# santurini/vsrlab

Hardware: AMD Instinct MI355X
Metric: LR frames/sec fwd+bwd, BasicVSR 4x 540p 7-frame clip, 1->8 MI355X (higher is better)
Workload: dtype bf16; 1 GPU; BasicVSR(mid=64,res_blocks=30,x4) fwd+Charbonnier+bwd+clip+Adam, 540x960->2160x3840, 7-frame clip, 2 clips per GPU (BASELINE configs[1]); clips_per_gpu=2, frames=7, res_blocks=30, parallelism=single GPU, arena=full, train_flow=False, trunk_chains=True

## Files before the change

vsrlab_amd/_lib.py:

```python
import ctypes
import os
from ctypes import c_char_p, c_float, c_int, c_longlong, c_size_t, c_void_p

_HERE = os.path.dirname(os.path.abspath(__file__))
LIB_PATH = os.environ.get("VSRLAB_AMD_LIB") or os.path.join(_HERE, "lib", "libvsrlab_hip.so")

DT_F32 = 0
DT_BF16 = 1


class BasicVSRDesc(ctypes.Structure):
    _fields_ = [("n", c_int), ("t", c_int), ("h", c_int), ("w", c_int), ("mid_channels", c_int),
                ("res_blocks", c_int), ("upscale", c_int), ("dtype", c_int), ("arena_mode", c_int)]


class DiscDesc(ctypes.Structure):
    _fields_ = [("n", c_int), ("h", c_int), ("w", c_int), ("mid_ch", c_int), ("dtype", c_int)]


class PerceptualDesc(ctypes.Structure):
    _fields_ = [("n", c_int), ("h", c_int), ("w", c_int), ("dtype", c_int), ("need_grad", c_int)]


class AttnDesc(ctypes.Structure):
# ... 101 lines not shown
    "vsr_raft_corr_lookup_fwd": (c_int, [ctypes.POINTER(RaftCorrDesc), _P, c_size_t, _P, _P, _P]),
    "vsr_raft_corr_lookup_bwd": (c_int, [ctypes.POINTER(RaftCorrDesc), _P, c_size_t, _P, _P, _P, c_size_t, _P]),
}
EXPORTS = tuple(_SIGNATURES)

OTHER_DEBUG_EXPORTS = ("vsr_debug_chain_inject_error", "vsr_debug_chain_item", "vsr_debug_chain_timeouts", "vsr_debug_chain_timing_begin",
                       "vsr_debug_chain_timing_read", "vsr_debug_warp_bwd_gather", "vsr_debug_warp_bwd_gather_c")
_LL = c_longlong
DEBUG_SIGNATURES = {
    "vsr_debug_tail_last2_fwd": (c_int, [c_int, _P, _P, _P, _P, _P, _P, _LL, _P, _P, _LL, c_int, c_int, c_int, c_int, c_int, c_int, c_int, _P]),
    "vsr_debug_tail_last2_dgrad": (c_int, [_P, _LL, _P, _P, c_int, _P, c_int, c_float, _P, c_int, c_int, c_int, _P]),
    "vsr_debug_tail_planar_c64": (c_int, [c_int, _P, _LL, c_int, _P, _P, _P, _P, c_int, c_float, _P, c_int, c_int, c_int, c_int, _P]),
    "vsr_debug_tail_last2_wgrad": (c_int, [c_int, _P, _P, _LL, c_int, _P, _P, _P, c_int, c_int, c_int, _P]),
    "vsr_debug_tail_conv_unshuffle": (c_int, [c_int, _P, _P, _P, c_int, _P, _P, c_int, c_int, c_int, _P]),
    "vsr_debug_tail_ps_dgrad": (c_int, [c_int, _P, _P, _P, _P, _P, c_int, c_int, _P, c_int, c_int, c_int, c_int, c_int, _P]),
    "vsr_debug_tail_ps_wgrads": (c_int, [c_int, _P, _P, c_int, _P, _P, _P, c_int, c_int, c_int, _P]),
    "vsr_debug_trunk_conv": (c_int, [c_int, c_int, c_int, c_int, _P, _P, _P, _P, _P, c_int, c_float, _P, _P, c_int, _P, _P, c_int, c_int,
                                     c_int, c_int, c_int, _P]),
    "vsr_debug_trunk_stem": (c_int, [c_int, c_int, c_int, _P, _P, _LL, _P, _P, _P, _P, c_int, c_float, c_int, c_int, c_int, _P]),
    "vsr_debug_trunk_stem_dgrad": (c_int, [c_int, c_int, c_int, _P, _P, _P, _P, _P, _LL, c_int, c_int, c_int, c_int, _P]),
    "vsr_debug_trunk_point": (c_int, [c_int, c_int, c_int, _P, _P, _P, _P, _P, _P, _P, c_int, c_int, c_int, _P]),
    "vsr_debug_trunk_wgrad_cc": (c_int, [c_int, c_int, c_int, _P, _P, c_int, _P, c_int, c_int, _P, c_int, _P, c_int, c_int, c_int, _P]),
    "vsr_debug_trunk_stem_wgrads": (c_int, [c_int, c_int, c_int, _P, _LL, _P, c_int, _P, _P, c_int, _P, _P, c_int, _P, c_int, c_int, c_int, _P]),
    "vsr_debug_trunk_chain": (c_int, [c_int, c_int, _P, _P, _P, c_int, _P, c_int, c_int, c_int, c_int, _P]),
    "vsr_debug_spy_conv": (c_int, [c_int, c_int, _P, _P, _P, _P, _P, c_int, _P, c_int, c_int, c_int, _P]),
    "vsr_debug_spy_dgrad": (c_int, [c_int, c_int, _P, _P, _P, _P, _P, c_int, c_int, c_int, _P]),
    "vsr_debug_spy_wgrad": (c_int, [c_int, c_int, _P, _P, _P, _P, c_int, _P, c_int, c_int, c_int, _P]),
    "vsr_debug_spy_prepare": (c_int, [c_int, _P, _P, _P, _P, c_int, c_int, c_int, c_int, c_int, c_int, c_int, _P]),
    "vsr_debug_spy_prepare_bwd": (c_int, [c_int, _P, _P, _P, _P, _P, _P, c_int, c_int, c_int, c_int, c_int, c_int, _P]),
    "vsr_debug_spy_dres": (c_int, [c_int, _P, _P, _P, c_int, c_int, c_int, _P]),
    "vsr_debug_spy_planar": (c_int, [c_int, _P, _P, _P, _P, _P, _LL, c_int, c_int, c_int, c_int, _P]),
}

SPATIAL_CORR_LIB_PATH = os.path.join(_HERE, "lib", "libvsrlab_spatial_corr.so")
SPATIAL_CORR_SIGNATURES = {
    "vsr_spatial_corr_workspace_bytes": (c_size_t, [ctypes.POINTER(SpatialCorrDesc)]),
    "vsr_spatial_corr_fwd": (c_int, [ctypes.POINTER(SpatialCorrDesc), _P, _P, _P, _P, c_size_t, _P]),
    "vsr_spatial_corr_bwd": (c_int, [ctypes.POINTER(SpatialCorrDesc), _P, _P, _P, _P, _P, _P, c_size_t, _P]),
}
SPATIAL_CORR_EXPORTS = tuple(SPATIAL_CORR_SIGNATURES)

JPEG_LIB_PATH = os.path.join(_HERE, "lib", "libvsrlab_jpeg.so")
JPEG_SIGNATURES = {
    "vsr_jpeg_workspace_bytes": (c_size_t, [ctypes.POINTER(JpegDesc)]),
    "vsr_jpeg_fwd": (c_int, [ctypes.POINTER(JpegDesc), _P, _P, _P, c_size_t, _P]),
}
JPEG_EXPORTS = tuple(JPEG_SIGNATURES)

WARP_TAPS_LIB_PATH = os.path.join(_HERE, "lib", "libvsrlab_warp_taps.so")
WARP_TAPS_SIGNATURES = {
    "vsr_warp_taps_fwd": (c_int, [ctypes.POINTER(WarpTapsDesc), _P, _P, _P, _P]),
    "vsr_warp_taps_bwd": (c_int, [ctypes.POINTER(WarpTapsDesc), _P, _P, _P, _P, _P]),
    "vsr_warp_taps_clip_fwd": (c_int, [ctypes.POINTER(WarpTapsDesc), _P, _P, _P, _P, _P]),
    "vsr_warp_taps_clip_bwd": (c_int, [ctypes.POINTER(WarpTapsDesc), _P, _P, _P, _P, _P, _P]),
}
WARP_TAPS_EXPORTS = tuple(WARP_TAPS_SIGNATURES)

_lib = None
_spatial_corr_lib = None
_jpeg_lib = None
_warp_taps_lib = None


def load_warp_taps():
    global _warp_taps_lib
    if _warp_taps_lib is None:
        if not os.path.exists(WARP_TAPS_LIB_PATH):
            raise RuntimeError(
                f"vsrlab_amd: HIP library not built ({WARP_TAPS_LIB_PATH} missing). Run "
                "`python -c 'import __graft_entry__ as g; g.build()'` or `make -C vsrlab_amd/csrc`.")
        lib = ctypes.CDLL(WARP_TAPS_LIB_PATH)
        for name, (res, args) in WARP_TAPS_SIGNATURES.items():
            fn = getattr(lib, name)
            fn.restype = res
            fn.argtypes = args
        _warp_taps_lib = lib
    return _warp_taps_lib


def load_jpeg():
    global _jpeg_lib
    if _jpeg_lib is None:
        if not os.path.exists(JPEG_LIB_PATH):
            raise RuntimeError(
                f"vsrlab_amd: HIP library not built ({JPEG_LIB_PATH} missing). Run "
                "`python -c 'import __graft_entry__ as g; g.build()'` or `make -C vsrlab_amd/csrc`.")
        lib = ctypes.CDLL(JPEG_LIB_PATH)
        for name, (res, args) in JPEG_SIGNATURES.items():
            fn = getattr(lib, name)
            fn.restype = res
            fn.argtypes = args
        _jpeg_lib = lib
    return _jpeg_lib

# ... 43 lines not shown
```

vsrlab_amd/csrc/conv3x3_persist.hip:

```cpp
#include "conv3x3_c64_tile.h"
#include <type_traits>

namespace {

constexpr int P_LDS = BIAS_OFF + 256;

__device__ uint4 g_conv_zero_chunk[2];

template <int ACT> __device__ __forceinline__ float p_act(float v, float slope) {
    if (ACT == ACT_RELU) return v > 0.f ? v : 0.f;
    if (ACT == ACT_LEAKY) return v > 0.f ? v : slope * v;
    return v;
}

#ifdef VSR_CLOCK
__device__ unsigned long long g_clk[256 * 4];
#endif

__device__ __forceinline__ void tile_coords(int tile, int ntx, int nty, int& n, int& ty0, int& tx0) {
    const int per = ntx * nty;
    n = tile / per;
    const int r = tile - n * per;
    const int ty = r / ntx;
    ty0 = ty * PTH;
    tx0 = (r - ty * ntx) * PTW;
}

struct TileIter {
    int tile, n, ty, tx;
    int sn, sty, stx;
    __device__ __forceinline__ void init(int first, int stride, int ntx, int nty) {
        const int per = ntx * nty;
        tile = first; n = first / per; int r = first - n * per; ty = r / ntx; tx = r - ty * ntx;
        sn = stride / per; r = stride - sn * per; sty = r / ntx; stx = r - sty * ntx;
    }
    __device__ __forceinline__ void advance(int stride, int ntx, int nty) {
        tile += stride;
        tx += stx; if (tx >= ntx) { tx -= ntx; ++ty; }
        ty += sty; if (ty >= nty) { ty -= nty; ++n; }
        n += sn;
    }
};

__device__ __forceinline__ float bf_lo(unsigned w) { return __uint_as_float(w << 16); }
__device__ __forceinline__ float bf_hi(unsigned w) { return __uint_as_float(w & 0xffff0000u); }

constexpr int DMA_PLAIN = 0;

template <int ACT, bool HAS_RES, int MASK>
__global__ __launch_bounds__(PNT, 1) void conv3x3_c64_persist_kernel(const ConvArgs ka) {
    extern __shared__ __attribute__((aligned(16))) char smem[];

    const int z = blockIdx.y;
    struct {
        int N, H, W, Ws, Wd, in_step, out_step, src_ox0, src_oy0, out_oxz, out_oyz, bias_zstride, unshuffle;
        long long src_nstride0, dst_nstride, w_zstride, plane;
        unsigned long long src0, wpack, resz, auxz, sign_bitsz, dstz, sign_outz, bias; float leaky_slope;
    } a = {ka.N, ka.H, ka.W, ka.Ws, ka.Wd, ka.in_step, ka.out_step, ka.src_ox[0], ka.src_oy[0], ka.out_ox[z], ka.out_oy[z], ka.bias_zstride, ka.unshuffle,
           ka.src_nstride[0], ka.dst_nstride, ka.w_zstride, ka.unshuffle_plane,
           (unsigned long long)ka.src[0], (unsigned long long)ka.wpack, (unsigned long long)ka.res[z], (unsigned long long)ka.aux[z],
           (unsigned long long)ka.sign_bits[z], (unsigned long long)ka.dst[z], (unsigned long long)ka.sign_out[z], (unsigned long long)ka.bias, ka.leaky_slope};
    asm volatile("" : "+s"(a.N), "+s"(a.H), "+s"(a.W), "+s"(a.Ws), "+s"(a.Wd), "+s"(a.in_step), "+s"(a.out_step), "+s"(a.src_ox0), "+s"(a.src_oy0),
                 "+s"(a.out_oxz), "+s"(a.out_oyz), "+s"(a.bias_zstride), "+s"(a.unshuffle), "+s"(a.src_nstride0), "+s"(a.dst_nstride), "+s"(a.w_zstride), "+s"(a.plane));
    asm volatile("" : "+s"(a.src0), "+s"(a.wpack), "+s"(a.resz), "+s"(a.auxz), "+s"(a.sign_bitsz), "+s"(a.dstz), "+s"(a.sign_outz), "+s"(a.bias), "+s"(a.leaky_slope));
    const int tid = threadIdx.x, lane = tid & 63, wave = tid >> 6;
    const int role = __builtin_amdgcn_readfirstlane(wave >> 2);
    const int w4 = wave & 3;
    const int l15 = lane & 15, q = lane >> 4;
    const int pxl = PM_LANE_PIXEL(l15);
    char* lds_w = smem;
    char* lds_t = smem + W_BYTES;
#ifdef VSR_CLOCK
    unsigned long long clk_t0 = 0, clk_r0 = 0;
    if (tid == 0) { clk_t0 = __builtin_amdgcn_s_memtime(); clk_r0 = __builtin_amdgcn_s_memrealtime(); }
#endif

    const int ntx = cdiv(a.W, PTW), nty = cdiv(a.H, PTH);
    const int total = a.N * ntx * nty;
    const int WSs = pm_ws(a.Ws), WSd = pm_ws(a.Wd);
    const TileWalk walk = xcd_tile_walk(total, blockIdx.x, gridDim.x);

    if (tid < 64) reinterpret_cast<float*>(smem + BIAS_OFF)[tid] = a.bias ? GP(const float, a.bias)[(long long)z * a.bias_zstride + pm_acc_chan(tid >> 4, tid & 15)] : 0.f;

    const auto* wg = GP(const u32x4_t, a.wpack + (unsigned long long)((long long)z * a.w_zstride) * 2);

    if (role == 1) {
        const auto* src = GP(const char, a.src0);
        const auto* zsrc = GP(const char, g_conv_zero_chunk);
        int rel[NPIECE_W];
        C64_DMA_REL(rel, w4, lane, a.in_step, a.src_oy0, a.src_ox0, WSs)
        auto issue = [&](const TileIter& it, int buf) {
            const int n = it.n, ty0 = it.ty * PTH, tx0 = it.tx * PTW;
            const auto* org = src + ((long long)n * a.src_nstride0 + pm_off(ty0 * a.in_step, tx0 * a.in_step, 0, a.Ws, 64)) * 2;
            char* dstb = lds_t + buf * IN_BYTES;
            C64_DMA_TILE(DMA_PLAIN, rel, org, zsrc, dstb, w4, lane, ty0, tx0, a.H, a.W)
        };
        int cur = 0;
        TileIter it;
        it.init(walk.first, walk.stride, ntx, nty);
        if (it.tile < walk.end) issue(it, 0);
        asm volatile("s_waitcnt vmcnt(0)" ::: "memory");
        __syncthreads();
        while (it.tile < walk.end) {
            it.advance(walk.stride, ntx, nty);
            if (it.tile < walk.end) issue(it, cur ^ 1);
            asm volatile("s_waitcnt vmcnt(0)" ::: "memory");
            __syncthreads();
            cur ^= 1;
        }
    } else {
        u32x4_t wv[WCH];
        C64_W_LOAD(wv, wg, tid)
        C64_MFMA_LANE(w4, l15, q, pxl)
        int loff[4];
#pragma unroll
        for (int nb = 0; nb < 4; ++nb) {
            const int dx = ((nb & 1) * 16 + pxl) * a.out_step + a.out_oxz;
            loff[nb] = ((((w4 * 2 + (nb >> 1)) * a.out_step) * WSd + (dx >> 5)) * 8 + q) * 256 + (dx & 31) * 8;
            if (a.unshuffle) {
                const int row = w4 * 2 + (nb >> 1), px = (nb & 1) * 16 + pxl;
                loff[nb] = (int)(((row & 1) * 2 + (px & 1)) * a.plane) + (((row >> 1) * pm_ws(a.Wd >> 1)) * 8 + q) * 256 + (px >> 1) * 8;
            }
        }
        C64_W_STORE(wv, lds_w, tid)
        asm volatile("s_waitcnt vmcnt(0)" ::: "memory");
        __syncthreads();
        auto* const dst_z = GP(bf16_t, a.dstz);
        const auto* const res_z = GP(const bf16_t, a.resz);
        const auto* const aux_z = GP(const bf16_t, a.auxz);
        const auto* const sbits_z = GP(const u32x2_t, a.sign_bitsz);
        auto* const sout_z = GP(u32x2_t, a.sign_outz);
        const float slope = vsr_slope(a.leaky_slope);

        f32x4_t bvec[4];
#pragma unroll
        for (int mb = 0; mb < 4; ++mb) bvec[mb] = c64_bias_rows(smem, q, mb);
        C64_RES_IDENTITY(idA, l15, q)
        static_assert(!HAS_RES || ACT == ACT_NONE, "the residual goes in on the matrix cores, ahead of any activation");

        int cur = 0;
        TileIter it;
        for (it.init(walk.first, walk.stride, ntx, nty); it.tile < walk.end; it.advance(walk.stride, ntx, nty)) {
            const int tile = it.tile, n = it.n, ty0 = it.ty * PTH, tx0 = it.tx * PTW;
            const long long tbase = a.unshuffle ? (long long)n * a.dst_nstride + pm_off(ty0 >> 1, tx0 >> 1, 0, a.Wd >> 1, 64)
                                                : (long long)n * a.dst_nstride + pm_off(ty0 * a.out_step + a.out_oyz, tx0 * a.out_step, 0, a.Wd, 64);
            const bool full = ty0 + PTH <= a.H && tx0 + PTW <= a.W;
            bool ok[4];
            constexpr bool BITS = MASK == MASK_RELU_BITS || MASK == MASK_LEAKY_BITS;
            constexpr bool LATE_MASK = HAS_RES && MASK != MASK_NONE && !BITS;
            u32x4_t rr[2][4], mm[2][4];
            u32x2_t sbits = {0u, 0u};
            if (BITS) sbits = sbits_z[c64_sign_word(tile, w4, lane)];
#pragma unroll
            for (int nb = 0; nb < 4; ++nb) ok[nb] = (tx0 + (nb & 1) * 16 + pxl < a.W) && (ty0 + w4 * 2 + (nb >> 1) < a.H);
#define CV_OPERANDS(OKN)                                                                                               \
            _Pragma("unroll") for (int nb = 0; nb < 4; ++nb) {                                                         \
                if (OKN) {                                                                                             \
                    _Pragma("unroll") for (int k = 0; k < 2; ++k) {                                                    \
                        const long long o = tbase + loff[nb] + k * 1024;                                               \
                        if (HAS_RES) rr[k][nb] = *GP(const u32x4_t, res_z + o);                                        \
                        if (MASK != MASK_NONE && !LATE_MASK && !BITS) mm[k][nb] = *GP(const u32x4_t, aux_z + o);       \
                    }                                                                                                  \
                }                                                                                                      \
            }
            if (HAS_RES || (MASK != MASK_NONE && !LATE_MASK && !BITS)) {
                if (full) { CV_OPERANDS(true) } else { CV_OPERANDS(ok[nb]) }
            }
#undef CV_OPERANDS

            f32x4_t acc[4][4];

            C64_K_LOOP(acc, bvec, cur)

            if (HAS_RES || MASK != MASK_NONE) __builtin_amdgcn_s_waitcnt(0x0F70);
            if constexpr (HAS_RES) { C64_ADD_RESIDUAL(acc, idA, rr) }
            unsigned sout[2] = {0u, 0u};
            auto epilogue = [&](auto FULL) {
#pragma unroll
            for (int nb = 0; nb < 4; ++nb) {
                if (decltype(FULL)::value || ok[nb]) {
                    auto* dst = dst_z + tbase + loff[nb];
#pragma unroll
                    for (int k = 0; k < 2; ++k) {
                        float v[8];
#pragma unroll
                        for (int j = 0; j < 4; ++j) { v[j] = acc[2 * k][nb][j]; v[4 + j] = acc[2 * k + 1][nb][j]; }
                        const unsigned wbits = k ? sbits.y : sbits.x;
                        unsigned ow[4];
                        if (ACT == ACT_RELU && !HAS_RES && MASK == MASK_NONE) {
                            C64_ARM_RELU(ow, v, nb, sout[k])
                        } else if (ACT == ACT_LEAKY && !HAS_RES && MASK == MASK_NONE) {
#pragma unroll
                            for (int jj = 0; jj < 4; ++jj) {
                                ow[jj] = pk_bf16(fmaxf(v[2 * jj], v[2 * jj] * slope), fmaxf(v[2 * jj + 1], v[2 * jj + 1] * slope));
                                sout[k] |= pk_min_u16(pk_max_i16(ow[jj], 0u), C64_K11) << (4 * nb + jj);
                            }
                        } else if (ACT == ACT_NONE && !HAS_RES && MASK == MASK_RELU_BITS) {
                            C64_ARM_MASKED(ow, v, nb, wbits)
                        } else {
#pragma unroll
                            for (int j = 0; j < 8; ++j) v[j] = p_act<ACT>(v[j], slope);
                            if (ACT != ACT_NONE && !HAS_RES) {
#pragma unroll
                                for (int j = 0; j < 8; ++j) sout[k] |= (v[j] > 0.f ? 1u : 0u) << (4 * nb + (j >> 1) + 16 * (j & 1));
                            }
                            if (BITS) {
                                const float neg = MASK == MASK_LEAKY_BITS ? slope : 0.f;
#pragma unroll
// ... 35 lines not shown
    }
#endif
}

__global__ void sign_bits_c64_kernel(const bf16_t* __restrict__ x, uint2* __restrict__ bits, int N, int H, int W) {
    const int ntx = cdiv(W, PTW), nty = cdiv(H, PTH);
    const long long total = (long long)N * ntx * nty * 256;
    const long long gid = (long long)blockIdx.x * blockDim.x + threadIdx.x;
    if (gid >= total) return;
    const int lane = (int)(gid & 63), w4 = (int)((gid >> 6) & 3);
    const int tile = (int)(gid >> 8);
    const int l15 = lane & 15, q = lane >> 4;
    const int pxl = PM_LANE_PIXEL(l15);
    int n, ty0, tx0;
    tile_coords(tile, ntx, nty, n, ty0, tx0);
    unsigned out[2] = {0u, 0u};
#pragma unroll
    for (int nb = 0; nb < 4; ++nb) {
        const int yy = ty0 + 2 * w4 + (nb >> 1), xx = tx0 + (nb & 1) * 16 + pxl;
        if (yy < H && xx < W) {
#pragma unroll
            for (int k = 0; k < 2; ++k) {
                const uint4 v = *reinterpret_cast<const uint4*>(x + (long long)n * pm_image_elems(H, W, 64) + pm_off(yy, xx, 4 * k + q, W, 64));
                const unsigned vw[4] = {v.x, v.y, v.z, v.w};
#pragma unroll
                for (int jj = 0; jj < 4; ++jj)
                    out[k] |= ((bf_lo(vw[jj]) > 0.f ? 1u : 0u) | (bf_hi(vw[jj]) > 0.f ? 0x10000u : 0u)) << (4 * nb + jj);
            }
        }
    }
    bits[gid] = make_uint2(out[0], out[1]);
}

template <int ACT, bool HAS_RES, int MASK>
static int launch_persist(const ConvArgs& a, int num_cus, hipStream_t st) {
    auto kern = conv3x3_c64_persist_kernel<ACT, HAS_RES, MASK>;
    static VsrDevOnce once;
    { const int rc = vsr_set_max_dynamic_lds(once, reinterpret_cast<const void*>(kern), P_LDS); if (rc != VSR_OK) return rc; }
    const int tiles = a.N * cdiv(a.W, PTW) * cdiv(a.H, PTH);
    int gx = num_cus / a.nz;
    gx &= ~7;
    if (gx < 8) gx = num_cus / a.nz;
    if (gx < 1) gx = 1;
    if (gx > tiles) gx = tiles;
    hipLaunchKernelGGL(kern, dim3(gx, a.nz), dim3(PNT), P_LDS, st, a);
    HIP_CHECK_RET(hipGetLastError());
    return VSR_OK;
}

}

#ifdef VSR_CLOCK
extern "C" int vsr_debug_read_clk(unsigned long long* host_out) {
    return hipMemcpyFromSymbol(host_out, HIP_SYMBOL(g_clk), sizeof(unsigned long long) * 256 * 4) == hipSuccess ? 0 : -3;
}
#endif

int vsr_launch_conv3x3_c64_persist(const ConvArgs& a, int num_cus, hipStream_t st) {
    bool res = false, aux = false;
    for (int z = 0; z < a.nz; ++z) { res = res || a.res[z]; aux = aux || a.aux[z]; }
    for (int z = 0; z < a.nz; ++z) if ((res && !a.res[z]) || (aux && !a.aux[z])) return VSR_ERR_UNSUPPORTED;
    int mask = aux ? a.mask_mode : MASK_NONE;
    if (mask == MASK_RELU && !res) {
        bool bits = true;
        for (int z = 0; z < a.nz; ++z) bits = bits && a.sign_bits[z];
        if (bits) mask = MASK_RELU_BITS;
    }
    if (mask == MASK_LEAKY && res) {
        bool bits = true;
        for (int z = 0; z < a.nz; ++z) bits = bits && a.sign_bits[z];
        if (bits) mask = MASK_LEAKY_BITS;
    }
    if (pm_image_elems((PTHH + 2) * a.in_step, a.Ws, 64) * 2 > 0x7fffffffLL || pm_image_elems(2 * PTH + 2, a.Wd, 64) > 0x7fffffffLL)
        return VSR_ERR_UNSUPPORTED;
    if (a.unshuffle) {
        if (a.nz != 1 || a.out_step != 1 || a.out_ox[0] || a.out_oy[0] || (a.Hd & 1) || (a.Wd & 1) || a.Hd != a.H || a.Wd != a.W || aux ||
            a.unshuffle_plane < (long long)a.N * pm_image_elems(a.Hd / 2, a.Wd / 2, 64) || a.dst_nstride != pm_image_elems(a.Hd / 2, a.Wd / 2, 64) ||
            3 * a.unshuffle_plane + pm_image_elems(PTH + 2, a.Wd / 2, 64) > 0x7fffffffLL)
            return VSR_ERR_UNSUPPORTED;
    }
#define PERSIST_CASE(ACT, RES, MASK) if (a.act == ACT && res == RES && mask == MASK) return launch_persist<ACT, RES, MASK>(a, num_cus, st);
    PERSIST_CASE(ACT_RELU, false, MASK_NONE)
    PERSIST_CASE(ACT_NONE, true, MASK_NONE)
    PERSIST_CASE(ACT_LEAKY, false, MASK_NONE)
    PERSIST_CASE(ACT_NONE, false, MASK_NONE)
    PERSIST_CASE(ACT_NONE, false, MASK_RELU)
    PERSIST_CASE(ACT_NONE, false, MASK_RELU_BITS)
    PERSIST_CASE(ACT_NONE, true, MASK_LEAKY)
    PERSIST_CASE(ACT_NONE, true, MASK_LEAKY_BITS)
    PERSIST_CASE(ACT_NONE, false, MASK_LEAKY)
#undef PERSIST_CASE
    return VSR_ERR_UNSUPPORTED;
}

int vsr_launch_sign_bits_c64(const void* x_pm, void* bits, int N, int H, int W, hipStream_t st) {
    if (!x_pm || !bits || N < 1 || H < 1 || W < 1) return VSR_ERR_BADARG;
    const long long total = (long long)N * cdiv(W, PTW) * cdiv(H, PTH) * 256;
    hipLaunchKernelGGL(sign_bits_c64_kernel, dim3((unsigned)((total + 255) / 256)), dim3(256), 0, st, (const bf16_t*)x_pm, (uint2*)bits, N, H, W);
    HIP_CHECK_RET(hipGetLastError());
    return VSR_OK;
}
```

vsrlab_amd/csrc/conv_mfma.hip:

```cpp
#include <cstdlib>
#include "elt.h"

namespace {

__device__ uint4 g_cm_zero[4];

constexpr int TW = 32;
constexpr int RW = 2;
constexpr int TH = 4 * RW;
constexpr int NTHREADS = 256;

typedef __attribute__((ext_vector_type(4))) unsigned cu32x4_t;
typedef __attribute__((ext_vector_type(8))) unsigned cu32x8_t;
template <typename T> struct RegChunk;
template <> struct RegChunk<bf16_t> { typedef cu32x4_t chunk_t; };
template <> struct RegChunk<float> { typedef cu32x8_t chunk_t; };
__device__ __forceinline__ cu32x4_t reg_chunk3(float a, float b, float c, bf16_t*) {
    union { bf16_t h[8]; cu32x4_t u; } t;
    t.u = cu32x4_t{0u, 0u, 0u, 0u};
    t.h[0] = (bf16_t)a; t.h[1] = (bf16_t)b; t.h[2] = (bf16_t)c;
    return t.u;
}
__device__ __forceinline__ cu32x8_t reg_chunk3(float a, float b, float c, float*) {
    return cu32x8_t{__float_as_uint(a), __float_as_uint(b), __float_as_uint(c), 0u, 0u, 0u, 0u, 0u};
// ... 362 lines not shown

#define VSR_CONV_SHAPES(X)                  \
    X(3, 1, 64, 64, false, 64, EPI_NHWC)     \
    X(3, 2, 64, 16, true, 64, EPI_NHWC)      \
    X(3, 1, 16, 16, true, 64, EPI_NHWC)      \
    X(3, 1, 64, 64, false, 32, EPI_PLANAR)   \
    X(3, 4, 64, 64, false, 64, EPI_NHWC)     \
    X(1, 2, 64, 64, false, 64, EPI_NHWC)     \
    X(1, 1, 64, 64, false, 64, EPI_NHWC)     \
    X(7, 1, 16, 16, false, 32, EPI_NHWC)     \
    X(7, 1, 32, 32, false, 64, EPI_NHWC)     \
    X(7, 1, 64, 64, false, 32, EPI_NHWC)     \
    X(7, 1, 32, 32, false, 32, EPI_NHWC)    \
    X(7, 1, 16, 16, false, 32, EPI_PLANAR)   \
     \
    X(3, 1, 16, 16, false, 32, EPI_NHWC)     \
    X(3, 1, 32, 32, false, 32, EPI_NHWC)     \
    X(3, 2, 16, 16, true, 32, EPI_NHWC)      \
    X(3, 2, 32, 16, true, 32, EPI_NHWC)      \
    X(3, 1, 16, 16, true, 32, EPI_NHWC)      \
    X(1, 2, 16, 16, false, 32, EPI_NHWC)     \
    X(1, 2, 32, 32, false, 32, EPI_NHWC)    \
    X(1, 1, 16, 16, false, 32, EPI_NHWC)     \
    X(1, 1, 32, 32, false, 32, EPI_NHWC)    \
    X(3, 4, 16, 16, false, 32, EPI_NHWC)     \
    X(3, 4, 32, 32, false, 32, EPI_NHWC)    \
    X(3, 1, 16, 16, false, 64, EPI_NHWC)     \
    X(3, 1, 32, 32, false, 64, EPI_NHWC)    \
    X(3, 1, 64, 64, false, 32, EPI_NHWC)     \
    X(3, 1, 16, 16, false, 32, EPI_PLANAR)   \
    X(3, 1, 32, 32, false, 32, EPI_PLANAR)

int vsr_launch_conv3x3_c64_persist(const ConvArgs& a, int num_cus, hipStream_t st);
int vsr_launch_c64_to_planar(const ConvArgs& a, hipStream_t st);
int vsr_launch_planar_c64_conv(const ConvArgs& a, hipStream_t st);
int vsr_launch_conv7x7_persist(const ConvArgs& a, int cin, int cop, int epi, int num_cus, hipStream_t st);

static bool vsr_force_generic_conv() { return vsr_env().generic_conv; }

int vsr_launch_conv(int dtype, int ks, int nsrc, int ca, int cb, int last_planar, int cout_t, int epi,
                    const ConvArgs& a, hipStream_t st) {
    if (a.N <= 0 || a.H <= 0 || a.W <= 0 || a.nz < 1 || a.nz > VSR_MAX_Z) return VSR_ERR_BADARG;
    if (dtype == VSR_BF16 && ks == 3 && nsrc == 1 && ca == 64 && cb == 64 && !last_planar && cout_t == 64 && epi == EPI_NHWC &&
        ((a.in_step == 1 && a.src_oy[0] == 0 && a.src_ox[0] == 0 && a.Hs == a.H && a.Ws == a.W) ||
         (a.in_step == 2 && a.Hs == 2 * a.H && a.Ws == 2 * a.W && (unsigned)a.src_oy[0] < 2u && (unsigned)a.src_ox[0] < 2u)) &&
        a.CD == 64 && a.cout_real == 64 &&
        a.src[0] != nullptr && !vsr_force_generic_conv()) {
        const int ps = vsr_launch_conv3x3_c64_persist(a, vsr_num_cus(), st);
        if (ps != VSR_ERR_UNSUPPORTED) return ps;
    }
    if (a.unshuffle) return VSR_ERR_UNSUPPORTED;
    if (dtype == VSR_BF16 && ks == 3 && nsrc == 1 && ca == 64 && cb == 64 && !last_planar && cout_t == 32 && epi == EPI_PLANAR &&
        !vsr_force_generic_conv()) {
        const int ps = vsr_launch_c64_to_planar(a, st);
        if (ps != VSR_ERR_UNSUPPORTED) return ps;
    }
    if (dtype == VSR_BF16 && ks == 3 && nsrc == 1 && last_planar && ca == 16 && cb == 16 && cout_t == 64 && epi == EPI_NHWC && !vsr_force_generic_conv()) {
        const int ps = vsr_launch_planar_c64_conv(a, st);
        if (ps != VSR_ERR_UNSUPPORTED) return ps;
    }
    if (dtype == VSR_BF16 && ks == 7 && nsrc == 1 && ca == cb && !last_planar && !vsr_force_generic_conv()) {
        const int ps = vsr_launch_conv7x7_persist(a, ca, cout_t, epi, vsr_num_cus(), st);
        if (ps != VSR_ERR_UNSUPPORTED) return ps;
    }
#define X(KS, NSRC, CA, CB, LP, COUT, EPI)                                                             \
    if (ks == KS && nsrc == NSRC && ca == CA && cb == CB && (last_planar != 0) == LP && cout_t == COUT && epi == EPI) { \
        if (dtype == VSR_BF16) return launch_inst<bf16_t, KS, NSRC, CA, CB, LP, COUT, EPI>(a, st);    \
        if (dtype == VSR_F32) return launch_inst<float, KS, NSRC, CA, CB, LP, COUT, EPI>(a, st);      \
        return VSR_ERR_BADARG;                                                                        \
    }
    VSR_CONV_SHAPES(X)
#undef X
    return VSR_ERR_UNSUPPORTED;
}
```

vsrlab_amd/csrc/engine.hip:

```cpp
#include <vector>
#include "recipes.h"
#include "spynet_engine.h"

namespace {

struct Plan {
    VsrBasicVSRDesc d = {};
    int C = 64, CO = 64;
    bool sb = false;
    bool bwd = false, flowgrad = false;
    bool diet = false;
    int rb = 0, n = 0, t = 0, h = 0, w = 0, dtype = VSR_F32;
    int scale = 4, ups = 2;
    bool unsh = false;
    size_t es = 4;
    size_t px1 = 0;
    size_t s_elems = 0;
    size_t stem_w[2] = {}, stem_wd[2] = {}, stem_b[2] = {};
    std::vector<size_t> blk_w[2], blk_wd[2], blk_b[2];
    size_t point_w = 0, point_wd = 0, point_b = 0;
    size_t up_w[2] = {}, up_wd[2] = {}, up_b[2] = {};
    size_t last0_w = 0, last0_wd = 0, last0_b = 0, last2_w = 0, last2_wd = 0, last2_b = 0;
    SpyPlan spy;
    size_t flows = 0;
// ... 236 lines not shown
}
int trunk_chain_forward(const Ctx& c, const Plan& p, int dir, int i) {
    ChainArgs a = {};
    a.base = c.ws; a.sync = (unsigned*)c.at(p.chain_sync[dir]); a.N = p.n; a.H = p.h; a.W = p.w; a.nlayers = 2 * p.rb;
    for (int b = 0; b < p.rb; ++b) {
        ChainLayer& l1 = a.layer[2 * b];
        l1 = {chain_off(p.xoff(dir, i, b)), chain_off(p.aoff(dir, i, b)), 0xffffffffu, 0xffffffffu, chain_off(p.sboff(dir, i, b)),
              chain_off(p.blk_w[dir][2 * b]), chain_off(p.blk_b[dir][2 * b]), CHAIN_RELU};
        ChainLayer& l2 = a.layer[2 * b + 1];
        l2 = {chain_off(p.aoff(dir, i, b)), chain_off(p.xoff(dir, i, b + 1)), chain_off(p.xoff(dir, i, b)), 0xffffffffu, 0xffffffffu,
              chain_off(p.blk_w[dir][2 * b + 1]), chain_off(p.blk_b[dir][2 * b + 1]), CHAIN_SKIP};
    }
    return chain_launch(a, c.st);
}
int trunk_chain_backward(const Ctx& c, const Plan& p, int dir, int i) {
    ChainArgs a = {};
    a.base = c.ws; a.sync = (unsigned*)c.at(p.chain_sync[dir]); a.N = p.n; a.H = p.h; a.W = p.w;
    int L = 0;
    for (int b = p.rb - 1; b >= 0; --b) {
        a.layer[L++] = {chain_off(p.dxoff(dir, i, b + 1)), chain_off(p.g1off(dir, i, b)), 0xffffffffu, chain_off(p.sboff(dir, i, b)), 0xffffffffu,
                        chain_off(p.blk_wd[dir][2 * b + 1]), 0xffffffffu, CHAIN_MASK};
        if (b > 0)
            a.layer[L++] = {chain_off(p.g1off(dir, i, b)), chain_off(p.dxoff(dir, i, b)), chain_off(p.dxoff(dir, i, b + 1)), 0xffffffffu, 0xffffffffu,
                            chain_off(p.blk_wd[dir][2 * b]), 0xffffffffu, CHAIN_SKIP};
    }
    a.nlayers = L;
    return chain_launch(a, c.st);
}

int trunk_forward(const Ctx& c, const Plan& p, int dir, int i, const void* warped, const float* lrs) {
    const int n = p.n, h = p.h, w = p.w, rb = p.rb;
    void* x = p.bwd ? c.at(p.xoff(dir, i, 0)) : c.at(p.feat[dir][i]);
    {
        CK(c.stem(true, warped, lrs + (size_t)i * 3 * h * w, (long long)p.t * 3 * h * w, c.at(p.stem_w[dir]), c.fat(p.stem_b[dir]), x, ACT_LEAKY, 0.f, n, h, w));
        if (p.sb) CK(vsr_launch_sign_bits_c64(x, c.at(p.SBX0[dir][i]), n, h, w, c.st));
    }
    if (chain_on(p)) return trunk_chain_forward(c, p, dir, i);
    for (int b = 0; b < rb; ++b) {
        void* act = p.bwd ? c.at(p.aoff(dir, i, b)) : c.at(p.scratchA[dir]);
        void* xn = p.bwd ? c.at(p.xoff(dir, i, b + 1)) : x;
        CK(c.conv(3, x, c.at(p.blk_w[dir][2 * b]), c.fat(p.blk_b[dir][2 * b]), act, ACT_RELU, nullptr, nullptr, 0, n, h, w,
                    p.sb ? c.at(p.sboff(dir, i, b)) : nullptr));
        CK(c.conv(3, act, c.at(p.blk_w[dir][2 * b + 1]), c.fat(p.blk_b[dir][2 * b + 1]), xn, ACT_NONE, x, nullptr, 0, n, h, w));
        x = xn;
    }
    return VSR_OK;
}

int last0_forward(const Ctx& c, const Plan& p, int i, void* sign_out) {
    const int S = p.scale;
    if (p.C == 64)
        return c.conv(3, c.at(p.U1[i]), c.at(p.last0_w), c.fat(p.last0_b), c.at(p.C0[i]), ACT_LEAKY, nullptr, nullptr, 0, p.n, S * p.h, S * p.w, sign_out);
    ConvArgs a = conv_args(p.n, S * p.h, S * p.w, c.C);
    a.src[0] = c.at(p.U1[i]); a.wpack = c.at(p.last0_w); a.bias = c.fat(p.last0_b); a.dst[0] = c.at(p.C0[i]); a.act = ACT_LEAKY;
    a.CD = 64; a.cout_real = 64; a.dst_nstride = pm_image_elems(S * p.h, S * p.w, 64);
    return vsr_launch_conv(c.dtype, 3, 1, p.C, p.C, 0, 64, EPI_NHWC, a, c.st);
}

int recon_forward(const Ctx& c, const Plan& p, int i, const float* lrs, float* sr) {
    const int n = p.n, h = p.h, w = p.w;
    CK(c.point_conv(c.at(p.feat[0][i]), c.at(p.feat[1][i]), c.at(p.point_w), c.fat(p.point_b), c.at(p.Pt[i]), n, h, w));
    if (p.sb) CK(vsr_launch_sign_bits_c64(c.at(p.Pt[i]), c.at(p.SBPt[i]), n, h, w, c.st));
    const int S = p.scale;
    CK(c.conv_ps(c.at(p.Pt[i]), c.at(p.up_w[0]), c.fat(p.up_b[0]), c.at(p.U0[i]), n, h, w));
    if (p.ups == 2) CK(c.conv_ps(c.at(p.U0[i]), c.at(p.up_w[1]), c.fat(p.up_b[1]), c.at(p.U1[i]), n, 2 * h, 2 * w));
    CK(last0_forward(c, p, i, p.sb ? c.at(p.SBC0[i]) : nullptr));
    {
        ConvArgs a = conv_args(n, S * h, S * w, c.C);
// ... 375 lines not shown
```

vsrlab_amd/csrc/recipes.h:

```cpp
#pragma once
#include <vector>
#include "host.h"

inline constexpr int NSPY = 5;
inline constexpr int SPY_CI[NSPY] = {8, 32, 64, 32, 16};
inline constexpr int SPY_CO[NSPY] = {32, 64, 32, 16, 2};
inline constexpr int SPY_CIP[NSPY] = {16, 32, 64, 32, 16};
inline constexpr int SPY_COP[NSPY] = {32, 64, 32, 32, 32};
inline constexpr int SPY_CD[NSPY] = {32, 64, 32, 16, 0};
inline constexpr int SPY_DK[NSPY] = {32, 64, 32, 16, 16};
inline constexpr int SPY_DROWS[NSPY] = {32, 32, 64, 32, 32};

struct Ctx {
    char* ws;
    hipStream_t st;
    int dtype;
    int C, CO;
    size_t es;
    float* slab;
    mutable std::vector<VsrPackDesc>* batch = nullptr;
    Ctx(char* ws_, hipStream_t st_, int dtype_, int C_ = 64, float* slab_ = nullptr)
        : ws(ws_), st(st_), dtype(dtype_), C(C_), CO(C_ < 32 ? 32 : C_), es(esize(dtype_)), slab(slab_) {}
    void* at(size_t off) const { return ws + off; }
    const float* fat(size_t off) const { return reinterpret_cast<const float*>(ws + off); }
// ... 51 lines not shown
                int rc = vsr_launch_conv(dtype, 3, 1, 64, 64, 0, 64, EPI_NHWC, a, st);
                if (rc != VSR_OK) return rc;
            }
            return VSR_OK;
        }
        ConvArgs a = conv_args(N, H, W, C);
        a.nz = 1; a.in_step = 2; a.Hs = 2 * H; a.Ws = 2 * W;
        for (int s = 0; s < 4; ++s) { a.src[s] = dy; a.src_oy[s] = s >> 1; a.src_ox[s] = s & 1; a.src_nstride[s] = pm_image_elems(2 * H, 2 * W, C); }
        a.wpack = wpackd; a.dst[0] = dx; a.aux[0] = aux; a.mask_mode = mask;
        return vsr_launch_conv(dtype, 3, 4, C, C, 0, CO, EPI_NHWC, a, st);
    }
    int ps_wgrads(const void* const* x, const void* const* dy, int nseg, bool dy_planes, int N, int H, int W, float* gw, float* gb, int accumulate) const {
        for (int z = 0; z < 4; ++z) {
            WgradArgs a = wg_base(N, H, W, C, C);
            a.nseg = nseg;
            for (int i = 0; i < nseg; ++i) {
                a.x[i] = x[i];
                a.dy[i] = dy_planes ? (const char*)dy[i] + (size_t)z * plane_elems(N, 2 * H, 2 * W) * es : dy[i];
            }
            if (!dy_planes) { a.dy_step = 2; a.dy_oy = z >> 1; a.dy_ox = z & 1; a.Hy = 2 * H; a.Wy = 2 * W; a.dy_nstride = pm_image_elems(2 * H, 2 * W, C); }
            CK(wgrad(a, {3, C, false, C, false}, {C, C, gw, C, 0, 4, z, gb, accumulate}));
        }
        return VSR_OK;
    }

    int pack_stem(const float* w, void* dst, bool cat) const {
        const int I_total = cat ? C + 3 : 3;
        if (cat) CK(pack(w, dst, 9, CO, C, C, C, I_total, 3, 1, 0, 0));
        return pack(w, (char*)dst + (cat ? (size_t)9 * CO * C * es : 0), 9, CO, 16, C, 3, I_total, 0, 1, 0, 0);
    }
    int pack_stem_dgrad(const float* w, void* dst) const { return pack(w, dst, 9, CO, C, C, C, C + 3, 3, 1, 0, 1); }
    int pack_stem_dlr(const float* w, void* dst, bool cat) const { return pack(w, dst, 9, 32, C, 3, C, cat ? C + 3 : 3, 0, 1, 0, 1); }
    int stem(bool cat, const void* feat, const float* lr, long long lr_nstride, const void* wpack, const float* bias, void* y, int act, float slope,
             int N, int H, int W) const {
        ConvArgs a = conv_args(N, H, W, C);
        a.wpack = wpack; a.bias = bias; a.dst[0] = y; a.act = act; a.leaky_slope = slope;
        a.src[cat ? 1 : 0] = lr; a.src_nstride[cat ? 1 : 0] = lr_nstride;
        if (!cat) return vsr_launch_conv(dtype, 3, 1, 16, 16, 1, CO, EPI_NHWC, a, st);
        a.src[0] = feat;
        return vsr_launch_conv(dtype, 3, 2, C, 16, 1, CO, EPI_NHWC, a, st);
    }
    int stem_wgrads(bool cat, WgradArgs& a_lr, WgradArgs& a_feat, float* gw, float* gb, int accumulate) const {
        const int I_total = cat ? C + 3 : 3;
        CK(wgrad(a_lr, {3, 16, true, C, false}, {C, 3, gw, I_total, 0, 1, 0, gb, accumulate}));
        if (cat && a_feat.nseg) CK(wgrad_cc(3, a_feat, gw, I_total, 3, nullptr, accumulate));
        return VSR_OK;
    }

    int pack_point(const float* w, void* dst, int mode) const {
        for (int s = 0; s < 2; ++s) CK(pack(w, (char*)dst + (size_t)s * CO * C * es, 1, CO, C, C, C, 2 * C, s * C, 1, 0, mode));
        return VSR_OK;
    }
    int point_conv(const void* xa, const void* xb, const void* wpack, const float* bias, void* y, int N, int H, int W) const {
        ConvArgs a = conv_args(N, H, W, C);
        a.src[0] = xa; a.src[1] = xb;
        a.wpack = wpack; a.bias = bias; a.dst[0] = y; a.act = ACT_LEAKY;
        return vsr_launch_conv(dtype, 1, 2, C, C, 0, CO, EPI_NHWC, a, st);
    }
    int point_dgrad(const void* dy, const void* wpackd, void* da, void* db, int N, int H, int W) const {
        ConvArgs a = conv_args(N, H, W, C);
        a.src[0] = dy; a.wpack = wpackd; a.w_zstride = CO * C; a.nz = 2;
        a.dst[0] = da; a.dst[1] = db;
        return vsr_launch_conv(dtype, 1, 1, C, C, 0, CO, EPI_NHWC, a, st);
    }

    int pack_spy(int j, const float* w, void* dst, int mode) const {
        if (mode == 0) return pack(w, dst, 49, SPY_COP[j], SPY_CIP[j], SPY_CO[j], SPY_CI[j], SPY_CI[j], 0, 1, 0, 0);
        return pack(w, dst, 49, SPY_DROWS[j], SPY_DK[j], SPY_CI[j], SPY_CO[j], SPY_CI[j], 0, 1, 0, 1);
    }
    int spy_conv(int j, const void* x, const void* wpack, const float* bias, void* y, int act, float slope, const float* pres, int N, int H, int W) const {
        ConvArgs a = conv_args(N, H, W, SPY_CD[j]);
        a.src[0] = x; a.src_nstride[0] = pm_image_elems(H, W, SPY_CIP[j]);
        a.wpack = wpack; a.bias = bias; a.act = act; a.leaky_slope = slope; a.cout_real = SPY_CO[j]; a.dst[0] = y;
// ... 52 lines not shown
```

Before: 57.90 LR frames/s.

## Route the BasicVSR stem conv through the persistent c64 kernel with fused LR operands

Adds a STEM variant of the persistent 3x3 c64 conv kernel. It reads the three planar LR channels straight from global memory, shuffles them across lanes with ds_bpermute, and feeds them to the matrix cores as one extra bf16 MFMA after the 64-channel feature K-loop, so the stem no longer goes through the generic two-source conv. The sign-bit output is passed into the stem launch so it can be written in the epilogue instead of by a separate sign_bits kernel. This adds per-tile uncoalesced LR loads, lane permutes and extra MFMAs, and it relies on strict shape guards that fall back to the generic path.

```diff
diff --git a/vsrlab_amd/_lib.py b/vsrlab_amd/_lib.py
--- a/vsrlab_amd/_lib.py
+++ b/vsrlab_amd/_lib.py
@@ -157,6 +157,12 @@
     "vsr_debug_spy_planar": (c_int, [c_int, _P, _P, _P, _P, _P, _LL, c_int, c_int, c_int, c_int, _P]),
 }
 
+STEM_HOOK_LIB_PATH = os.path.join(_HERE, "lib", "libvsrlab_hip_stem_hook.so")
+STEM_HOOK_SIGNATURES = {
+    "vsr_debug_trunk_stem_bits": (c_int, [c_int, c_int, c_int, _P, _P, _LL, _P, _P, _P, _P, c_int, c_float, _P, c_int, c_int, c_int, _P]),
+    "vsr_debug_trunk_conv": DEBUG_SIGNATURES["vsr_debug_trunk_conv"],
+}
+
 SPATIAL_CORR_LIB_PATH = os.path.join(_HERE, "lib", "libvsrlab_spatial_corr.so")
 SPATIAL_CORR_SIGNATURES = {
     "vsr_spatial_corr_workspace_bytes": (c_size_t, [ctypes.POINTER(SpatialCorrDesc)]),
@@ -185,6 +191,25 @@
 _spatial_corr_lib = None
 _jpeg_lib = None
 _warp_taps_lib = None
+
+
+_stem_hook_lib = None
+
+
+def load_stem_hook():
+    global _stem_hook_lib
+    if _stem_hook_lib is None:
+        if not os.path.exists(STEM_HOOK_LIB_PATH):
+            raise RuntimeError(
+                f"vsrlab_amd: test library not built ({STEM_HOOK_LIB_PATH} missing). Run "
+                "`python -c 'import __graft_entry__ as g; g.build()'` or `make -C vsrlab_amd/csrc`.")
+        lib = ctypes.CDLL(STEM_HOOK_LIB_PATH)
+        for name, (res, args) in STEM_HOOK_SIGNATURES.items():
+            fn = getattr(lib, name)
+            fn.restype = res
+            fn.argtypes = args
+        _stem_hook_lib = lib
+    return _stem_hook_lib
 
 
 def load_warp_taps():
diff --git a/vsrlab_amd/csrc/conv3x3_persist.hip b/vsrlab_amd/csrc/conv3x3_persist.hip
--- a/vsrlab_amd/csrc/conv3x3_persist.hip
+++ b/vsrlab_amd/csrc/conv3x3_persist.hip
@@ -47,7 +47,7 @@
 
 constexpr int DMA_PLAIN = 0;
 
-template <int ACT, bool HAS_RES, int MASK>
+template <int ACT, bool HAS_RES, int MASK, bool STEM = false>
 __global__ __launch_bounds__(PNT, 1) void conv3x3_c64_persist_kernel(const ConvArgs ka) {
     extern __shared__ __attribute__((aligned(16))) char smem[];
 
@@ -63,6 +63,12 @@
     asm volatile("" : "+s"(a.N), "+s"(a.H), "+s"(a.W), "+s"(a.Ws), "+s"(a.Wd), "+s"(a.in_step), "+s"(a.out_step), "+s"(a.src_ox0), "+s"(a.src_oy0),
                  "+s"(a.out_oxz), "+s"(a.out_oyz), "+s"(a.bias_zstride), "+s"(a.unshuffle), "+s"(a.src_nstride0), "+s"(a.dst_nstride), "+s"(a.w_zstride), "+s"(a.plane));
     asm volatile("" : "+s"(a.src0), "+s"(a.wpack), "+s"(a.resz), "+s"(a.auxz), "+s"(a.sign_bitsz), "+s"(a.dstz), "+s"(a.sign_outz), "+s"(a.bias), "+s"(a.leaky_slope));
+    unsigned long long lr_src = 0;
+    long long lr_nstride = 0;
+    if constexpr (STEM) {
+        lr_src = (unsigned long long)ka.src[1]; lr_nstride = ka.src_nstride[1];
+        asm volatile("" : "+s"(lr_src), "+s"(lr_nstride));
+    }
     const int tid = threadIdx.x, lane = tid & 63, wave = tid >> 6;
     const int role = __builtin_amdgcn_readfirstlane(wave >> 2);
     const int w4 = wave & 3;
@@ -93,6 +99,16 @@
             const int n = it.n, ty0 = it.ty * PTH, tx0 = it.tx * PTW;
             const auto* org = src + ((long long)n * a.src_nstride0 + pm_off(ty0 * a.in_step, tx0 * a.in_step, 0, a.Ws, 64)) * 2;
             char* dstb = lds_t + buf * IN_BYTES;
+            if constexpr (STEM) {
+                if (!a.src0) {
+#pragma unroll
+                    for (int i = 0; i < NPIECE_W; ++i) {
+                        const int piece = w4 + 4 * i;
+                        if (piece < NPIECE_T && piece * 64 + lane < IN_CHUNKS) C64_GLDS16(zsrc, dstb + piece * 1024, DMA_PLAIN);
+                    }
+                    return;
+                }
+            }
             C64_DMA_TILE(DMA_PLAIN, rel, org, zsrc, dstb, w4, lane, ty0, tx0, a.H, a.W)
         };
         int cur = 0;
@@ -111,6 +127,17 @@
     } else {
         u32x4_t wv[WCH];
         C64_W_LOAD(wv, wg, tid)
+        unsigned short lr_wraw[STEM ? 4 : 1][8];
+        if constexpr (STEM) {
+            const auto* wlr = GP(const unsigned short, a.wpack + 2ull * 9 * 64 * 64);
+#pragma unroll
+            for (int j = 0; j < 8; ++j) {
+                const bool used = q < 3 || j < 3;
+                const int tap = q < 3 ? (j / 3) * 3 + q : 6 + j, c = q < 3 ? j % 3 : 2;
+#pragma unroll
+                for (int mb = 0; mb < 4; ++mb) lr_wraw[mb][j] = wlr[used ? (tap * 64 + pm_acc_chan(mb, l15)) * 16 + c : 0];
+            }
+        }
         C64_MFMA_LANE(w4, l15, q, pxl)
         int loff[4];
 #pragma unroll
@@ -137,6 +164,26 @@
         for (int mb = 0; mb < 4; ++mb) bvec[mb] = c64_bias_rows(smem, q, mb);
         C64_RES_IDENTITY(idA, l15, q)
         static_assert(!HAS_RES || ACT == ACT_NONE, "the residual goes in on the matrix cores, ahead of any activation");
+        static_assert(!STEM || (!HAS_RES && MASK == MASK_NONE), "the stem's LR operands take the residual's registers");
+        u32x4_t lr_a[STEM ? 4 : 1];
+        const auto* const lr_zero = GP(const float, g_conv_zero_chunk);
+        const int w4u = __builtin_amdgcn_readfirstlane(w4);
+        int lr_bp[2], lr_bq[2];
+        if constexpr (STEM) {
+#pragma unroll
+            for (int mb = 0; mb < 4; ++mb) {
+                unsigned wd[4];
+#pragma unroll
+                for (int jj = 0; jj < 4; ++jj)
+                    wd[jj] = ((q < 3 || 2 * jj < 3) ? (unsigned)lr_wraw[mb][2 * jj] : 0u) | ((q < 3 || 2 * jj + 1 < 3) ? (unsigned)lr_wraw[mb][2 * jj + 1] << 16 : 0u);
+                lr_a[mb] = u32x4_t{wd[0], wd[1], wd[2], wd[3]};
+            }
+#pragma unroll
+            for (int hh = 0; hh < 2; ++hh) {
+                lr_bq[hh] = 4 * (16 * hh + pxl);
+                lr_bp[hh] = lr_bq[hh] + 4 * (q < 3 ? q : 0);
+            }
+        }
 
         int cur = 0;
         TileIter it;
@@ -167,13 +214,47 @@
                 if (full) { CV_OPERANDS(true) } else { CV_OPERANDS(ok[nb]) }
             }
 #undef CV_OPERANDS
+            float lr_row[STEM ? 4 : 1][3];
+            if constexpr (STEM) {
+                const unsigned long long lr_tb = lr_src + 4ull * (unsigned long long)((long long)n * lr_nstride + (long long)(ty0 + 2 * w4u - 1) * a.W + (tx0 - 1));
+                const bool col_in = lane < PTWH && (unsigned)(tx0 - 1 + lane) < (unsigned)a.W;
+#pragma unroll
+                for (int r = 0; r < 4; ++r) {
+                    const bool in = col_in && (unsigned)(ty0 + 2 * w4u - 1 + r) < (unsigned)a.H;
+#pragma unroll
+                    for (int c = 0; c < 3; ++c) {
+                        const unsigned long long brc = lr_tb + 4ull * (unsigned long long)((long long)c * a.H * a.W + (long long)r * a.W);
+                        lr_row[r][c] = *(in ? GP(const float, brc + 4u * (unsigned)lane) : lr_zero);
+                    }
+                }
+            }
 
             f32x4_t acc[4][4];
 
             C64_K_LOOP(acc, bvec, cur)
 
-            if (HAS_RES || MASK != MASK_NONE) __builtin_amdgcn_s_waitcnt(0x0F70);
+            if (HAS_RES || MASK != MASK_NONE || STEM) __builtin_amdgcn_s_waitcnt(0x0F70);
             if constexpr (HAS_RES) { C64_ADD_RESIDUAL(acc, idA, rr) }
+            if constexpr (STEM) {
+#pragma unroll
+                for (int nb = 0; nb < 4; ++nb) {
+                    float lr_v[8];
+#pragma unroll
+                    for (int j = 0; j < 8; ++j) {
+                        const int got = __builtin_amdgcn_ds_bpermute(lr_bp[nb & 1], __builtin_bit_cast(int, lr_row[(nb >> 1) + j / 3][j % 3]));
+                        int v = q < 3 ? got : 0;
+                        if (j < 3) {
+                            const int g3 = __builtin_amdgcn_ds_bpermute(lr_bq[nb & 1] + 4 * j, __builtin_bit_cast(int, lr_row[(nb >> 1) + 2][2]));
+                            v = q < 3 ? got : g3;
+                        }
+                        lr_v[j] = __builtin_bit_cast(float, v);
+                    }
+                    const u32x4_t b = {pk_bf16(lr_v[0], lr_v[1]), pk_bf16(lr_v[2], lr_v[3]), pk_bf16(lr_v[4], lr_v[5]), pk_bf16(lr_v[6], lr_v[7])};
+#pragma unroll
+                    for (int mb = 0; mb < 4; ++mb)
+                        acc[mb][nb] = __builtin_amdgcn_mfma_f32_16x16x32_bf16(__builtin_bit_cast(bf16x8_t, lr_a[mb]), __builtin_bit_cast(bf16x8_t, b), acc[mb][nb], 0, 0, 0);
+                }
+            }
             unsigned sout[2] = {0u, 0u};
             auto epilogue = [&](auto FULL) {
 #pragma unroll
@@ -275,9 +356,9 @@
     bits[gid] = make_uint2(out[0], out[1]);
 }
 
-template <int ACT, bool HAS_RES, int MASK>
+template <int ACT, bool HAS_RES, int MASK, bool STEM = false>
 static int launch_persist(const ConvArgs& a, int num_cus, hipStream_t st) {
-    auto kern = conv3x3_c64_persist_kernel<ACT, HAS_RES, MASK>;
+    auto kern = conv3x3_c64_persist_kernel<ACT, HAS_RES, MASK, STEM>;
     static VsrDevOnce once;
     { const int rc = vsr_set_max_dynamic_lds(once, reinterpret_cast<const void*>(kern), P_LDS); if (rc != VSR_OK) return rc; }
     const int tiles = a.N * cdiv(a.W, PTW) * cdiv(a.H, PTH);
@@ -336,6 +417,19 @@
     return VSR_ERR_UNSUPPORTED;
 }
 
+int vsr_launch_conv3x3_c64_stem(const ConvArgs& a, int num_cus, hipStream_t st) {
+    if (a.nz != 1 || a.in_step != 1 || a.out_step != 1 || a.Hs != a.H || a.Ws != a.W || a.Hd != a.H || a.Wd != a.W || a.CD != 64 || a.cout_real != 64 ||
+        a.src_oy[0] || a.src_ox[0] || a.src_oy[1] || a.src_ox[1] || a.out_oy[0] || a.out_ox[0] || a.res[0] || a.aux[0] || a.unshuffle || a.pres ||
+        (a.planar_c && a.planar_c != 3) || !a.src[1] || !a.wpack || !a.dst[0] || a.src_nstride[1] < 3LL * a.H * a.W)
+        return VSR_ERR_UNSUPPORTED;
+    if (pm_image_elems(PTHH + 2, a.Ws, 64) * 2 > 0x7fffffffLL || pm_image_elems(2 * PTH + 2, a.Wd, 64) > 0x7fffffffLL ||
+        (3LL * a.H * a.W + 2LL * a.W + 64) * 4 > 0x7fffffffLL)
+        return VSR_ERR_UNSUPPORTED;
+    if (a.act == ACT_LEAKY) return launch_persist<ACT_LEAKY, false, MASK_NONE, true>(a, num_cus, st);
+    if (a.act == ACT_NONE && !a.sign_out[0]) return launch_persist<ACT_NONE, false, MASK_NONE, true>(a, num_cus, st);
+    return VSR_ERR_UNSUPPORTED;
+}
+
 int vsr_launch_sign_bits_c64(const void* x_pm, void* bits, int N, int H, int W, hipStream_t st) {
     if (!x_pm || !bits || N < 1 || H < 1 || W < 1) return VSR_ERR_BADARG;
     const long long total = (long long)N * cdiv(W, PTW) * cdiv(H, PTH) * 256;
diff --git a/vsrlab_amd/csrc/conv_mfma.hip b/vsrlab_amd/csrc/conv_mfma.hip
--- a/vsrlab_amd/csrc/conv_mfma.hip
+++ b/vsrlab_amd/csrc/conv_mfma.hip
@@ -418,6 +418,7 @@
     X(3, 1, 32, 32, false, 32, EPI_PLANAR)
 
 int vsr_launch_conv3x3_c64_persist(const ConvArgs& a, int num_cus, hipStream_t st);
+int vsr_launch_conv3x3_c64_stem(const ConvArgs& a, int num_cus, hipStream_t st);
 int vsr_launch_c64_to_planar(const ConvArgs& a, hipStream_t st);
 int vsr_launch_planar_c64_conv(const ConvArgs& a, hipStream_t st);
 int vsr_launch_conv7x7_persist(const ConvArgs& a, int cin, int cop, int epi, int num_cus, hipStream_t st);
@@ -435,6 +436,10 @@
         const int ps = vsr_launch_conv3x3_c64_persist(a, vsr_num_cus(), st);
         if (ps != VSR_ERR_UNSUPPORTED) return ps;
     }
+    if (dtype == VSR_BF16 && ks == 3 && nsrc == 2 && ca == 64 && cb == 16 && last_planar && cout_t == 64 && epi == EPI_NHWC && !vsr_force_generic_conv()) {
+        const int ps = vsr_launch_conv3x3_c64_stem(a, vsr_num_cus(), st);
+        if (ps != VSR_ERR_UNSUPPORTED || a.sign_out[0]) return ps;
+    }
     if (a.unshuffle) return VSR_ERR_UNSUPPORTED;
     if (dtype == VSR_BF16 && ks == 3 && nsrc == 1 && ca == 64 && cb == 64 && !last_planar && cout_t == 32 && epi == EPI_PLANAR &&
         !vsr_force_generic_conv()) {
diff --git a/vsrlab_amd/csrc/engine.hip b/vsrlab_amd/csrc/engine.hip
--- a/vsrlab_amd/csrc/engine.hip
+++ b/vsrlab_amd/csrc/engine.hip
@@ -292,8 +292,8 @@
     const int n = p.n, h = p.h, w = p.w, rb = p.rb;
     void* x = p.bwd ? c.at(p.xoff(dir, i, 0)) : c.at(p.feat[dir][i]);
     {
-        CK(c.stem(true, warped, lrs + (size_t)i * 3 * h * w, (long long)p.t * 3 * h * w, c.at(p.stem_w[dir]), c.fat(p.stem_b[dir]), x, ACT_LEAKY, 0.f, n, h, w));
-        if (p.sb) CK(vsr_launch_sign_bits_c64(x, c.at(p.SBX0[dir][i]), n, h, w, c.st));
+        CK(c.stem(true, warped, lrs + (size_t)i * 3 * h * w, (long long)p.t * 3 * h * w, c.at(p.stem_w[dir]), c.fat(p.stem_b[dir]), x, ACT_LEAKY, 0.f, n, h, w,
+                  p.sb ? c.at(p.SBX0[dir][i]) : nullptr));
     }
     if (chain_on(p)) return trunk_chain_forward(c, p, dir, i);
     for (int b = 0; b < rb; ++b) {
diff --git a/vsrlab_amd/csrc/recipes.h b/vsrlab_amd/csrc/recipes.h
--- a/vsrlab_amd/csrc/recipes.h
+++ b/vsrlab_amd/csrc/recipes.h
@@ -107,13 +107,20 @@
     int pack_stem_dgrad(const float* w, void* dst) const { return pack(w, dst, 9, CO, C, C, C, C + 3, 3, 1, 0, 1); }
     int pack_stem_dlr(const float* w, void* dst, bool cat) const { return pack(w, dst, 9, 32, C, 3, C, cat ? C + 3 : 3, 0, 1, 0, 1); }
     int stem(bool cat, const void* feat, const float* lr, long long lr_nstride, const void* wpack, const float* bias, void* y, int act, float slope,
-             int N, int H, int W) const {
-        ConvArgs a = conv_args(N, H, W, C);
-        a.wpack = wpack; a.bias = bias; a.dst[0] = y; a.act = act; a.leaky_slope = slope;
+             int N, int H, int W, void* sign_out = nullptr) const {
+        if (sign_out && (dtype != VSR_BF16 || C != 64)) return VSR_ERR_UNSUPPORTED;
+        ConvArgs a = conv_args(N, H, W, C);
+        a.wpack = wpack; a.bias = bias; a.dst[0] = y; a.act = act; a.leaky_slope = slope; a.sign_out[0] = sign_out;
         a.src[cat ? 1 : 0] = lr; a.src_nstride[cat ? 1 : 0] = lr_nstride;
-        if (!cat) return vsr_launch_conv(dtype, 3, 1, 16, 16, 1, CO, EPI_NHWC, a, st);
-        a.src[0] = feat;
-        return vsr_launch_conv(dtype, 3, 2, C, 16, 1, CO, EPI_NHWC, a, st);
+        int rc;
+        if (!cat) {
+            rc = vsr_launch_conv(dtype, 3, 1, 16, 16, 1, CO, EPI_NHWC, a, st);
+        } else {
+            a.src[0] = feat;
+            rc = vsr_launch_conv(dtype, 3, 2, C, 16, 1, CO, EPI_NHWC, a, st);
+        }
+        if (rc == VSR_OK && sign_out && (!cat || vsr_env().generic_conv)) return vsr_launch_sign_bits_c64(y, sign_out, N, H, W, st);
+        return rc;
     }
     int stem_wgrads(bool cat, WgradArgs& a_lr, WgradArgs& a_feat, float* gw, float* gb, int accumulate) const {
         const int I_total = cat ? C + 3 : 3;
diff --git a/vsrlab_amd/csrc/trunk_stem_hook.hip b/vsrlab_amd/csrc/trunk_stem_hook.hip
--- /dev/null
+++ b/vsrlab_amd/csrc/trunk_stem_hook.hip
@@ -0,0 +1,16 @@
+#include "recipes.h"
+
+extern "C" {
+
+int vsr_debug_trunk_stem_bits(int dtype, int C, int cat, const void* feat_pm, const float* lr, long long lr_nstride, const float* w, const float* bias,
+                              void* wpack, void* y_pm, int act, float slope, void* sign_out, int N, int H, int W, void* stream) {
+    if (bad_dtype(dtype) || (C != 16 && C != 32 && C != 64) || (cat & ~1) || !lr || !wpack || !y_pm || bad_dims(N, H, W) ||
+        lr_nstride < (long long)3 * H * W || (act != ACT_NONE && act != ACT_LEAKY) || (!cat && feat_pm))
+        return VSR_ERR_BADARG;
+    if (sign_out && (dtype != VSR_BF16 || C != 64 || act == ACT_NONE)) return VSR_ERR_UNSUPPORTED;
+    const Ctx c(nullptr, (hipStream_t)stream, dtype, C);
+    if (w) CK(c.pack_stem(w, wpack, cat != 0));
+    return c.stem(cat != 0, feat_pm, lr, lr_nstride, wpack, bias, y_pm, act, slope, N, H, W, sign_out);
+}
+
+}
```

Result: no change. 58.23 LR frames/s, median of 6 (+0.6%).
